# ltronchin/LatentAugment

Measured on NVIDIA B200. Metric: augmented images/sec, higher is better.
Workload: dtype bf16 operands, f32 accumulate

## Files before the change

latentaugment_b200/csrc/kernels.cu:

```cuda
#include "kernels.cuh"

#include <cuda_bf16.h>

#include "act.cuh"
#include "sm100.cuh"

namespace la {

namespace {

__device__ __forceinline__ float warp_sum(float v) {
#pragma unroll
    for (int o = 16; o >= 1; o >>= 1) v += __shfl_xor_sync(0xffffffffu, v, o);
    return v;
}
__device__ __forceinline__ double warp_sum_d(double v) {
#pragma unroll
    for (int o = 16; o >= 1; o >>= 1) v += __shfl_xor_sync(0xffffffffu, v, o);
    return v;
}
__device__ __forceinline__ void split_store(__nv_bfloat16* hi, __nv_bfloat16* lo, long long i, float v) {
    const __nv_bfloat16 h = __float2bfloat16_rn(v);
    hi[i] = h;
    if (lo) lo[i] = __float2bfloat16_rn(v - __bfloat162float(h));
// ... 185 lines not shown
__global__ void const_modulate_kernel(const float* __restrict__ c_f32, const float* __restrict__ s0, int batch, int hw, int C,
                                      __nv_bfloat16* hi, __nv_bfloat16* lo) {
    const long long idx = blockIdx.x * static_cast<long long>(blockDim.x) + threadIdx.x;
    if (idx >= static_cast<long long>(batch) * hw * C) return;
    const int c = static_cast<int>(idx % C);
    const int p = static_cast<int>((idx / C) % hw);
    const int n = static_cast<int>(idx / (static_cast<long long>(C) * hw));
    split_store(hi, lo, idx, c_f32[p * C + c] * s0[static_cast<long long>(n) * C + c]);
}

__device__ __forceinline__ unsigned pack2(float a, float b) {
    __nv_bfloat162 v = __floats2bfloat162_rn(a, b);
    return *reinterpret_cast<unsigned*>(&v);
}
__device__ __forceinline__ void st_bf16x2(unsigned* hi, unsigned* lo, long long i, float a, float b) {
    hi[i] = pack2(a, b);
    if (lo) lo[i] = pack2(a - __bfloat162float(__float2bfloat16_rn(a)), b - __bfloat162float(__float2bfloat16_rn(b)));
}

constexpr int kFirSeg = 32;
template <bool FWD, bool SPLIT, bool SEP>
__global__ void __launch_bounds__(256, SEP ? 3 : 2) upfir_slide_kernel(const __grid_constant__ UpFirParams P, int cpb, int chan_blocks) {
    const int hc = P.C >> 1;
    const int rows_per_block = 256 / cpb;
    const int cb = blockIdx.z % chan_blocks, n = blockIdx.z / chan_blocks;
    const int cp = cb * cpb + threadIdx.x % cpb;
    const int r = blockIdx.y * rows_per_block + threadIdx.x / cpb;
    const int x0 = blockIdx.x * kFirSeg;
    const int TW = P.OW + 1;
    const int out_h = FWD ? P.OH : P.TH, out_w = FWD ? P.OW : TW, out_pitch = FWD ? P.OW : P.TWp;
    const int src_h = FWD ? P.TH : P.OH, src_w = FWD ? TW : P.OW, src_pitch = FWD ? P.TWp : P.OW;
    if (r >= out_h) return;
    const int org = FWD ? -1 : -2;
    const unsigned* sh = reinterpret_cast<const unsigned*>(FWD ? P.t_hi : P.gy_hi);
    const unsigned* sl = reinterpret_cast<const unsigned*>(FWD ? P.t_lo : P.gy_lo);
    float wk[16], wy[4], wx[4];
#pragma unroll
    for (int k = 0; k < 16; ++k) wk[k] = FWD ? P.fk[k] : P.fk[15 - k];
#pragma unroll
    for (int k = 0; k < 4; ++k) { wy[k] = FWD ? P.fy[k] : P.fy[3 - k]; wx[k] = FWD ? P.fx[k] : P.fx[3 - k]; }
    long long rowoff[4];
    float rowmask[4];
#pragma unroll
    for (int k = 0; k < 4; ++k) {
        const int sr = r + org + k;
        const bool ok = sr >= 0 && sr < src_h;
        rowoff[k] = ((static_cast<long long>(n) * src_h + (ok ? sr : 0)) * src_pitch) * hc + cp;
        rowmask[k] = ok ? 1.f : 0.f;
    }
    float2 win[SEP ? 1 : 4][7];
    auto load_col = [&](int slot, int sc) {
        const bool cok = sc >= 0 && sc < src_w;
        const long long coff = static_cast<long long>(cok ? sc : 0) * hc;
        unsigned u[4], l[4];
#pragma unroll
        for (int k = 0; k < 4; ++k) {
            u[k] = __ldg(sh + rowoff[k] + coff);
            if (SPLIT) l[k] = __ldg(sl + rowoff[k] + coff);
        }
        float2 colsum = make_float2(0.f, 0.f);
#pragma unroll
        for (int k = 0; k < 4; ++k) {
            float2 v = make_float2(__uint_as_float(u[k] << 16), __uint_as_float(u[k] & 0xffff0000u));
            if (SPLIT) { v.x += __uint_as_float(l[k] << 16); v.y += __uint_as_float(l[k] & 0xffff0000u); }
            if (SEP) {
                const float m = wy[k] * rowmask[k];
                colsum.x = fmaf(m, v.x, colsum.x);
                colsum.y = fmaf(m, v.y, colsum.y);
            } else {
                const float m = cok ? rowmask[k] : 0.f;
                win[k][slot] = make_float2(v.x * m, v.y * m);
            }
        }
        if (SEP) win[0][slot] = cok ? colsum : make_float2(0.f, 0.f);
    };
#pragma unroll
    for (int k = 0; k < 3; ++k) load_col(k, x0 + org + k);

    float2 dm = make_float2(0.f, 0.f), bs = dm, sn = dm;
    const float* nrow = nullptr;
    if (FWD && !P.act_saved) {
        const int c = 2 * cp;
        dm = __ldg(reinterpret_cast<const float2*>(P.demod + static_cast<long long>(n) * P.C + c));
        bs = __ldg(reinterpret_cast<const float2*>(P.bias + c));
        if (P.s_next) sn = __ldg(reinterpret_cast<const float2*>(P.s_next + static_cast<long long>(n) * P.C + c));
        if (P.noise) nrow = P.noise + n * P.noise_stride_n + static_cast<long long>(r) * P.OW;
    }
    unsigned* oh = reinterpret_cast<unsigned*>(FWD ? P.x_hi : P.gt_hi);
    unsigned* ol = SPLIT ? reinterpret_cast<unsigned*>(FWD ? P.x_lo : P.gt_lo) : nullptr;
    unsigned* xsh = reinterpret_cast<unsigned*>(P.xs_hi);
    unsigned* xsl = SPLIT ? reinterpret_cast<unsigned*>(P.xs_lo) : nullptr;
    const long long obase = ((static_cast<long long>(n) * out_h + r) * out_pitch) * hc + cp;

#pragma unroll 1
    for (int xb = 0; xb < kFirSeg; xb += 4) {
        if (x0 + xb >= out_w) break;
#pragma unroll
        for (int u = 0; u < 4; ++u) load_col(3 + u, x0 + xb + org + 3 + u);
        float nzv[4];
#pragma unroll
        for (int u = 0; u < 4; ++u) nzv[u] = (FWD && nrow && x0 + xb + u < out_w) ? __ldg(nrow + x0 + xb + u) * P.noise_scale : 0.f;
#pragma unroll
        for (int u = 0; u < 4; ++u) {
            const int x = x0 + xb + u;
            if (x >= out_w) continue;
            float a0 = 0.f, a1 = 0.f;
            if (SEP) {
#pragma unroll
                for (int kx = 0; kx < 4; ++kx) {
                    a0 = fmaf(wx[kx], win[0][u + kx].x, a0);
                    a1 = fmaf(wx[kx], win[0][u + kx].y, a1);
                }
            } else {
#pragma unroll
                for (int ky = 0; ky < 4; ++ky)
#pragma unroll
                    for (int kx = 0; kx < 4; ++kx) {
                        const float2 v = win[ky][u + kx];
                        a0 = fmaf(wk[ky * 4 + kx], v.x, a0);
                        a1 = fmaf(wk[ky * 4 + kx], v.y, a1);
                    }
            }
            const long long o = obase + static_cast<long long>(x) * hc;
            if (FWD && P.act_saved) {
                const unsigned sv = __ldg(reinterpret_cast<const unsigned*>(P.act_saved) + o);
                const unsigned svl = P.act_saved_lo ? __ldg(reinterpret_cast<const unsigned*>(P.act_saved_lo) + o) : 0u;
                const float s0 = __uint_as_float(sv << 16) + __uint_as_float(svl << 16);
                const float s1 = __uint_as_float(sv & 0xffff0000u) + __uint_as_float(svl & 0xffff0000u);
                const float thr = act_saved_clamp(P.act_clamp, P.act_saved_lo != nullptr);
                const float g0 = act_grad(a0 * P.act_gain, s0, P.act_slope, thr), g1 = act_grad(a1 * P.act_gain, s1, P.act_slope, thr);
                st_bf16x2(oh, ol, o, g0, g1);
            } else if (FWD) {
                float z0 = fmaf(a0, dm.x, nzv[u]) + bs.x, z1 = fmaf(a1, dm.y, nzv[u]) + bs.y;
                z0 = (z0 > 0.f ? z0 : z0 * P.act_slope) * P.act_gain;
                z1 = (z1 > 0.f ? z1 : z1 * P.act_slope) * P.act_gain;
                if (P.act_clamp >= 0.f) {
                    z0 = fminf(fmaxf(z0, -P.act_clamp), P.act_clamp);
                    z1 = fminf(fmaxf(z1, -P.act_clamp), P.act_clamp);
                }
                st_bf16x2(oh, ol, o, z0, z1);
                if (P.s_next) st_bf16x2(xsh, xsl, o, z0 * sn.x, z1 * sn.y);
            } else {
                st_bf16x2(oh, ol, o, a0, a1);
            }
        }
#pragma unroll
        for (int ky = 0; ky < (SEP ? 1 : 4); ++ky)
#pragma unroll
            for (int k = 0; k < 3; ++k) win[ky][k] = win[ky][4 + k];
    }
}

constexpr int kFirRing = 8, kFirStrip = 32, kFirSlotBytes = 4608, kFirInPx = 35;
template <bool FWD>
__global__ void __launch_bounds__(160) upfir_tma_kernel(const __grid_constant__ UpFirParams P, int rows_per_cta, int nslabs) {
    extern __shared__ __align__(128) uint8_t fsm[];
    uint8_t* ring = fsm;
    uint8_t* stage = fsm + kFirRing * kFirSlotBytes;
    uint64_t* full = reinterpret_cast<uint64_t*>(stage + 4 * 2 * 2 * 1024);
    uint64_t* empty = full + kFirRing;
    const int warp = threadIdx.x >> 5, lane = threadIdx.x & 31;
    const int slab = blockIdx.y % nslabs, rblk = blockIdx.y / nslabs;
    const int n = blockIdx.z;
    const int x0 = blockIdx.x * kFirStrip;
    const int out_h = FWD ? P.OH : P.TH;
    const int r0 = rblk * rows_per_cta, r1 = min(r0 + rows_per_cta, out_h);
    const int org = FWD ? -1 : -2;
    const int c0 = slab * 64;
    const CUtensorMap* in_map = FWD ? &P.fwd_in : &P.bwd_in;
    if (threadIdx.x == 0) {
        for (int s = 0; s < kFirRing; ++s) { mbar_init(&full[s], 1); mbar_init(&empty[s], 4); }
        fence_barrier_init();
        prefetch_tmap(in_map);
    }
    __syncthreads();
    const int nrows_in = (r1 - r0) + 3;
    if (warp == 4) {
        if (lane == 0) {
            for (int j = 0; j < nrows_in; ++j) {
                const int s = j % kFirRing;
                mbar_wait(&empty[s], ((j / kFirRing) & 1) ^ 1, nullptr, 0);
                mbar_expect_tx(&full[s], kFirInPx * 128);
                tma_load_4d(ring + s * kFirSlotBytes, in_map, &full[s], c0, x0 + org, r0 + org + j, n);
            }
        }
        return;
    }
    float wy[4], wx[4];
#pragma unroll
    for (int k = 0; k < 4; ++k) { wy[k] = FWD ? P.fy[k] : P.fy[3 - k]; wx[k] = FWD ? P.fx[k] : P.fx[3 - k]; }
    float2 dm = make_float2(0.f, 0.f), bs = dm, sn = dm;
    const int c = c0 + 2 * lane;
    if (FWD && !P.act_saved) {
        dm = __ldg(reinterpret_cast<const float2*>(P.demod + static_cast<long long>(n) * P.C + c));
        bs = __ldg(reinterpret_cast<const float2*>(P.bias + c));
        if (P.s_next) sn = __ldg(reinterpret_cast<const float2*>(P.s_next + static_cast<long long>(n) * P.C + c));
    }
    const float clampv = P.act_clamp >= 0.f ? P.act_clamp : __int_as_float(0x7f800000);
    const float saved_thr = act_saved_clamp(P.act_clamp, false);
    const int px0 = warp * 8;
    uint8_t* my_stage = stage + warp * 4096;
    if constexpr (!FWD) {
        float2 ha[8], hb[8], hc[8], hd[8];
        auto hpass = [&](int j, float2 (&h)[8]) {
            mbar_wait(&full[j % kFirRing], (j / kFirRing) & 1, nullptr, 0);
            const unsigned* row = reinterpret_cast<const unsigned*>(ring + (j % kFirRing) * kFirSlotBytes) + px0 * 32 + lane;
            float2 in[11];
#pragma unroll
            for (int q = 0; q < 11; ++q) {
                const unsigned u = row[q * 32];
                in[q] = make_float2(__uint_as_float(u << 16), __uint_as_float(u & 0xffff0000u));
            }
            __syncwarp();
            if (lane == 0) mbar_arrive(&empty[j % kFirRing]);
#pragma unroll
            for (int i = 0; i < 8; ++i) {
                float a0 = wx[0] * in[i].x, a1 = wx[0] * in[i].y;
#pragma unroll
                for (int k = 1; k < 4; ++k) { a0 = fmaf(wx[k], in[i + k].x, a0); a1 = fmaf(wx[k], in[i + k].y, a1); }
                h[i] = make_float2(a0, a1);
            }
        };
        auto out_row = [&](int r, const float2 (&h0)[8], const float2 (&h1)[8], const float2 (&h2)[8], float2 (&h3)[8]) {
            const int j0 = r - r0;
            hpass(j0 + 3, h3);
            float nzv[8];
            unsigned svv[8];
            if (FWD && P.act_saved) {
                const unsigned* sp = reinterpret_cast<const unsigned*>(P.act_saved) +
                                     ((static_cast<long long>(n) * P.OH + r) * P.OW) * (P.C >> 1) + (c0 >> 1) + lane;
#pragma unroll
                for (int i = 0; i < 8; ++i) {
                    const int x = x0 + px0 + i;
                    svv[i] = x < P.OW ? __ldg(sp + static_cast<long long>(x) * (P.C >> 1)) : 0u;
                }
            }
            if (FWD && P.noise && !P.act_saved) {
                const float4* np = reinterpret_cast<const float4*>(P.noise + n * P.noise_stride_n + static_cast<long long>(r) * P.OW + x0 + px0);
                const bool in = x0 + px0 + 8 <= P.OW;
                const float4 a = in ? __ldg(np) : make_float4(0.f, 0.f, 0.f, 0.f), b = in ? __ldg(np + 1) : a;
                nzv[0] = a.x; nzv[1] = a.y; nzv[2] = a.z; nzv[3] = a.w; nzv[4] = b.x; nzv[5] = b.y; nzv[6] = b.z; nzv[7] = b.w;
#pragma unroll
                for (int i = 0; i < 8; ++i) nzv[i] *= P.noise_scale;
            } else {
#pragma unroll
                for (int i = 0; i < 8; ++i) nzv[i] = 0.f;
            }
            uint8_t* sx = my_stage + (j0 & 1) * 2048;
            if (lane == 0) bulk_wait_read<1>();
            __syncwarp();
#pragma unroll
            for (int i = 0; i < 8; ++i) {
                const float a0 = fmaf(wy[3], h3[i].x, fmaf(wy[2], h2[i].x, fmaf(wy[1], h1[i].x, wy[0] * h0[i].x)));
                const float a1 = fmaf(wy[3], h3[i].y, fmaf(wy[2], h2[i].y, fmaf(wy[1], h1[i].y, wy[0] * h0[i].y)));
                if (FWD && P.act_saved) {
                    const float s0 = __uint_as_float(svv[i] << 16), s1 = __uint_as_float(svv[i] & 0xffff0000u);
                    const float g0 = act_grad(a0 * P.act_gain, s0, P.act_slope, saved_thr);
                    const float g1 = act_grad(a1 * P.act_gain, s1, P.act_slope, saved_thr);
                    reinterpret_cast<unsigned*>(sx)[i * 32 + lane] = pack2(g0, g1);
                } else if (FWD) {
                    float z0 = fmaf(a0, dm.x, nzv[i]) + bs.x, z1 = fmaf(a1, dm.y, nzv[i]) + bs.y;
                    z0 = (z0 > 0.f ? z0 : z0 * P.act_slope) * P.act_gain;
                    z1 = (z1 > 0.f ? z1 : z1 * P.act_slope) * P.act_gain;
                    z0 = fminf(fmaxf(z0, -clampv), clampv);
                    z1 = fminf(fmaxf(z1, -clampv), clampv);
                    reinterpret_cast<unsigned*>(sx)[i * 32 + lane] = pack2(z0, z1);
                    reinterpret_cast<unsigned*>(sx + 1024)[i * 32 + lane] = pack2(z0 * sn.x, z1 * sn.y);
                } else {
                    reinterpret_cast<unsigned*>(sx)[i * 32 + lane] = pack2(a0, a1);
                }
            }
            fence_proxy_async();
            __syncwarp();
            if (lane == 0) {
                if (FWD) {
                    tma_store_4d(&P.fwd_out_x, sx, c0, x0 + px0, r, n);
                    if (P.s_next && !P.act_saved) tma_store_4d(&P.fwd_out_xs, sx + 1024, c0, x0 + px0, r, n);
                } else {
                    tma_store_4d(&P.bwd_out, sx, c0, x0 + px0, r, n);
                }
                bulk_commit();
            }
        };
        if (r0 < r1) { hpass(0, ha); hpass(1, hb); hpass(2, hc); }
        for (int r = r0; r < r1; r += 4) {
            out_row(r, ha, hb, hc, hd);
            if (r + 1 < r1) out_row(r + 1, hb, hc, hd, ha);
            if (r + 2 < r1) out_row(r + 2, hc, hd, ha, hb);
            if (r + 3 < r1) out_row(r + 3, hd, ha, hb, hc);
        }
    } else {
        for (int j = 0; j < 3; ++j) mbar_wait(&full[j % kFirRing], (j / kFirRing) & 1, nullptr, 0);
        for (int r = r0; r < r1; ++r) {
            const int j0 = r - r0;
            mbar_wait(&full[(j0 + 3) % kFirRing], ((j0 + 3) / kFirRing) & 1, nullptr, 0);
            float2 cs[11];
#pragma unroll
            for (int q = 0; q < 11; ++q) cs[q] = make_float2(0.f, 0.f);
#pragma unroll
            for (int k = 0; k < 4; ++k) {
                const unsigned* row = reinterpret_cast<const unsigned*>(ring + ((j0 + k) % kFirRing) * kFirSlotBytes) + px0 * 32 + lane;
#pragma unroll
                for (int q = 0; q < 11; ++q) {
                    const unsigned u = row[q * 32];
                    cs[q].x = fmaf(wy[k], __uint_as_float(u << 16), cs[q].x);
                    cs[q].y = fmaf(wy[k], __uint_as_float(u & 0xffff0000u), cs[q].y);
                }
            }
            __syncwarp();
            if (lane == 0) mbar_arrive(&empty[j0 % kFirRing]);
            float nzv[8];
            unsigned svv[8];
            if (FWD && P.act_saved) {
                const unsigned* sp = reinterpret_cast<const unsigned*>(P.act_saved) +
                                     ((static_cast<long long>(n) * P.OH + r) * P.OW) * (P.C >> 1) + (c0 >> 1) + lane;
#pragma unroll
                for (int i = 0; i < 8; ++i) {
                    const int x = x0 + px0 + i;
                    svv[i] = x < P.OW ? __ldg(sp + static_cast<long long>(x) * (P.C >> 1)) : 0u;
                }
            }
            if (FWD && P.noise && !P.act_saved) {
                const float4* np = reinterpret_cast<const float4*>(P.noise + n * P.noise_stride_n + static_cast<long long>(r) * P.OW + x0 + px0);
                const bool in = x0 + px0 + 8 <= P.OW;
                const float4 a = in ? __ldg(np) : make_float4(0.f, 0.f, 0.f, 0.f), b = in ? __ldg(np + 1) : a;
                nzv[0] = a.x; nzv[1] = a.y; nzv[2] = a.z; nzv[3] = a.w; nzv[4] = b.x; nzv[5] = b.y; nzv[6] = b.z; nzv[7] = b.w;
#pragma unroll
                for (int i = 0; i < 8; ++i) nzv[i] *= P.noise_scale;
            } else {
#pragma unroll
                for (int i = 0; i < 8; ++i) nzv[i] = 0.f;
            }
            uint8_t* sx = my_stage + (j0 & 1) * 2048;
            if (lane == 0) bulk_wait_read<1>();
            __syncwarp();
#pragma unroll
            for (int i = 0; i < 8; ++i) {
                float a0 = 0.f, a1 = 0.f;
#pragma unroll
                for (int k = 0; k < 4; ++k) { a0 = fmaf(wx[k], cs[i + k].x, a0); a1 = fmaf(wx[k], cs[i + k].y, a1); }
                if (FWD && P.act_saved) {
                    const float s0 = __uint_as_float(svv[i] << 16), s1 = __uint_as_float(svv[i] & 0xffff0000u);
                    const float g0 = act_grad(a0 * P.act_gain, s0, P.act_slope, saved_thr);
                    const float g1 = act_grad(a1 * P.act_gain, s1, P.act_slope, saved_thr);
                    reinterpret_cast<unsigned*>(sx)[i * 32 + lane] = pack2(g0, g1);
                } else if (FWD) {
                    float z0 = fmaf(a0, dm.x, nzv[i]) + bs.x, z1 = fmaf(a1, dm.y, nzv[i]) + bs.y;
                    z0 = (z0 > 0.f ? z0 : z0 * P.act_slope) * P.act_gain;
                    z1 = (z1 > 0.f ? z1 : z1 * P.act_slope) * P.act_gain;
                    z0 = fminf(fmaxf(z0, -clampv), clampv);
                    z1 = fminf(fmaxf(z1, -clampv), clampv);
                    reinterpret_cast<unsigned*>(sx)[i * 32 + lane] = pack2(z0, z1);
                    reinterpret_cast<unsigned*>(sx + 1024)[i * 32 + lane] = pack2(z0 * sn.x, z1 * sn.y);
                } else {
                    reinterpret_cast<unsigned*>(sx)[i * 32 + lane] = pack2(a0, a1);
                }
            }
            fence_proxy_async();
            __syncwarp();
            if (lane == 0) {
                if (FWD) {
                    tma_store_4d(&P.fwd_out_x, sx, c0, x0 + px0, r, n);
                    if (P.s_next && !P.act_saved) tma_store_4d(&P.fwd_out_xs, sx + 1024, c0, x0 + px0, r, n);
                } else {
                    tma_store_4d(&P.bwd_out, sx, c0, x0 + px0, r, n);
                }
                bulk_commit();
            }
        }
    }
    if (lane == 0) bulk_wait_read<0>();
}

__device__ __forceinline__ void up_taps(int v, int lowres, int& i0, int& i1, float& c0, float& c1) {
    const int m = v >> 1;
    if (v & 1) { i0 = m; i1 = m + 1; c0 = 0.75f; c1 = 0.25f; }
    else { i0 = m - 1; i1 = m; c0 = 0.25f; c1 = 0.75f; }
    if (i0 < 0) { c0 = 0.f; i0 = 0; }
    if (i1 >= lowres) { c1 = 0.f; i1 = lowres - 1; }
}

__device__ __forceinline__ float4 f4_fma(float c, float4 a, float4 acc) {
    return make_float4(fmaf(c, a.x, acc.x), fmaf(c, a.y, acc.y), fmaf(c, a.z, acc.z), fmaf(c, a.w, acc.w));
}

__device__ __forceinline__ float4 rgb_preclamp(const float4* __restrict__ parts, int nparts, long long stride, long long pix,
                                               const float* __restrict__ bias, int img_c) {
    float4 t = make_float4(0.f, 0.f, 0.f, 0.f);
    for (int b = 0; b < nparts; ++b) {
        const float4 p = parts[b * stride + pix];
        t.x += p.x; t.y += p.y; t.z += p.z;
    }
    t.x += bias[0];
    if (img_c > 1) t.y += bias[1];
    if (img_c > 2) t.z += bias[2];
    return t;
}

__global__ void rgb_combine_kernel(const float4* __restrict__ parts, int nparts, const float* __restrict__ bias, int img_c,
                                   float clamp, const float4* __restrict__ img_low, int batch, int res, float4* img,
                                   float* out_nchw) {
    const long long pix = blockIdx.x * static_cast<long long>(blockDim.x) + threadIdx.x;
    const long long total = static_cast<long long>(batch) * res * res;
    if (pix >= total) return;
    float4 t = rgb_preclamp(parts, nparts, total, pix, bias, img_c);
    if (clamp >= 0.f) {
        t.x = fminf(fmaxf(t.x, -clamp), clamp);
        t.y = fminf(fmaxf(t.y, -clamp), clamp);
        t.z = fminf(fmaxf(t.z, -clamp), clamp);
    }
    const int w = static_cast<int>(pix % res), h = static_cast<int>((pix / res) % res);
    const int n = static_cast<int>(pix / (static_cast<long long>(res) * res));
    if (img_low) {
        const int lr = res >> 1;
        int y0, y1, x0, x1;
        float cy0, cy1, cx0, cx1;
        up_taps(h, lr, y0, y1, cy0, cy1);
        up_taps(w, lr, x0, x1, cx0, cx1);
        const float4* base = img_low + static_cast<long long>(n) * lr * lr;
        float4 u = make_float4(0.f, 0.f, 0.f, 0.f);
        u = f4_fma(cy0 * cx0, base[y0 * lr + x0], u);
        u = f4_fma(cy0 * cx1, base[y0 * lr + x1], u);
        u = f4_fma(cy1 * cx0, base[y1 * lr + x0], u);
        u = f4_fma(cy1 * cx1, base[y1 * lr + x1], u);
        t.x += u.x; t.y += u.y; t.z += u.z;
    }
    img[pix] = t;
    if (out_nchw) {
        const long long plane = static_cast<long long>(res) * res;
        float* o = out_nchw + static_cast<long long>(n) * img_c * plane + static_cast<long long>(h) * res + w;
        o[0] = t.x;
        if (img_c > 1) o[plane] = t.y;
        if (img_c > 2) o[2 * plane] = t.z;
    }
}

__global__ void rgb_backward_kernel(const float4* __restrict__ g_img, const float4* __restrict__ parts, int nparts,
                                    const float* __restrict__ bias, int img_c, float clamp, int batch, int res, float4* g_rgb,
                                    float4* g_img_low) {
    const long long pix = blockIdx.x * static_cast<long long>(blockDim.x) + threadIdx.x;
    const long long total = static_cast<long long>(batch) * res * res;
    if (pix >= total) return;
    const float4 g = g_img[pix];
    const float4 t = rgb_preclamp(parts, nparts, total, pix, bias, img_c);
    float4 r = g;
    if (clamp >= 0.f) {
        if (!(fabsf(t.x) <= clamp)) r.x = 0.f;
        if (!(fabsf(t.y) <= clamp)) r.y = 0.f;
        if (!(fabsf(t.z) <= clamp)) r.z = 0.f;
    }
    r.w = 0.f;
    g_rgb[pix] = r;
    if (g_img_low) {
        const int w = static_cast<int>(pix % res), h = static_cast<int>((pix / res) % res);
        if ((w | h) & 1) return;
        const int n = static_cast<int>(pix / (static_cast<long long>(res) * res));
        const int my = h >> 1, mx = w >> 1, lr = res >> 1;
        const float cf[4] = {0.25f, 0.75f, 0.75f, 0.25f};
        float4 acc = make_float4(0.f, 0.f, 0.f, 0.f);
        const float4* base = g_img + static_cast<long long>(n) * res * res;
        for (int a = 0; a < 4; ++a) {
            const int yy = 2 * my - 1 + a;
            if (yy < 0 || yy >= res) continue;
            for (int b = 0; b < 4; ++b) {
                const int xx = 2 * mx - 1 + b;
                if (xx < 0 || xx >= res) continue;
                acc = f4_fma(cf[a] * cf[b], base[static_cast<long long>(yy) * res + xx], acc);
            }
        }
        g_img_low[(static_cast<long long>(n) * lr + my) * lr + mx] = acc;
    }
}

__global__ void pix_loss_kernel(const float4* __restrict__ img, const float4* __restrict__ bank_mean, int batch, int res,
                                int img_c, int crop_off, int crop_size, float w_pix, float4* g_img, float* loss_parts) {
    const long long total = static_cast<long long>(batch) * res * res;
    const float gs = -(w_pix / img_c) * 2.f / (static_cast<float>(batch) * crop_size * crop_size);
    float acc = 0.f;
    for (long long pix = blockIdx.x * static_cast<long long>(blockDim.x) + threadIdx.x; pix < total;
         pix += static_cast<long long>(gridDim.x) * blockDim.x) {
        const int w = static_cast<int>(pix % res), h = static_cast<int>((pix / res) % res);
        float4 g = make_float4(0.f, 0.f, 0.f, 0.f);
        if (h >= crop_off && h < crop_off + crop_size && w >= crop_off && w < crop_off + crop_size) {
            const float4 x = img[pix];
            const float4 y = bank_mean[h * res + w];
            g.x = gs * (x.x - y.x);
            acc += x.x * x.x - 2.f * x.x * y.x;
            if (img_c > 1) { g.y = gs * (x.y - y.y); acc += x.y * x.y - 2.f * x.y * y.y; }
            if (img_c > 2) { g.z = gs * (x.z - y.z); acc += x.z * x.z - 2.f * x.z * y.z; }
        }
        g_img[pix] = g;
    }
    __shared__ float sm[32];
    acc = warp_sum(acc);
    if ((threadIdx.x & 31) == 0) sm[threadIdx.x >> 5] = acc;
    __syncthreads();
    if (threadIdx.x < 32) {
        float v = threadIdx.x < (blockDim.x >> 5) ? sm[threadIdx.x] : 0.f;
        v = warp_sum(v);
        if (threadIdx.x == 0) loss_parts[blockIdx.x] = v;
    }
}

__global__ void style_grad_rgb_kernel(LayerTable T, int batch, const float* __restrict__ red_rgb, float* g_s) {
    const RgbDesc D = T.rgb[blockIdx.y];
    const int i = blockIdx.x * blockDim.x + threadIdx.x;
    const int n = blockIdx.z;
    if (i >= D.cin) return;
    const float* rr = red_rgb + 3LL * batch * D.roff;
    const long long e = static_cast<long long>(n) * D.cin + i;
    const long long plane = static_cast<long long>(batch) * D.cin;
    float g = D.wt[i] * rr[e];
    if (D.img_c > 1) g += D.wt[D.cin + i] * rr[plane + e];
    if (D.img_c > 2) g += D.wt[2 * D.cin + i] * rr[2 * plane + e];
    g_s[static_cast<long long>(batch) * D.soff + e] = g;
}

constexpr int kGwRows = 64, kGwSamples = 4;
__global__ void gw_partial_kernel(const float* __restrict__ g_s, const float* __restrict__ a_cat, const int* __restrict__ chunk_soff,
                                  const int* __restrict__ chunk_cin, int batch, int w_dim, float* partial) {
// ... 99 lines not shown
    for (int k = threadIdx.x; k < w_dim; k += blockDim.x) {
        double acc = 0.0;
        for (int m = m0; m < m1; ++m)
            for (int j = 0; j < num_ws; ++j) {
                const double v = W[(static_cast<long long>(m) * num_ws + j) * w_dim + k];
                acc += v;
                sq += v * v;
            }
        psum[static_cast<long long>(blockIdx.x) * w_dim + k] = acc;
    }
    __shared__ double sm[32];
    sq = warp_sum_d(sq);
    if ((threadIdx.x & 31) == 0) sm[threadIdx.x >> 5] = sq;
    __syncthreads();
    if (threadIdx.x == 0) {
        double t = 0.0;
        for (int i = 0; i < (blockDim.x >> 5); ++i) t += sm[i];
        pm2[blockIdx.x] = t;
    }
}
__global__ void latent_bank_final_kernel(const double* __restrict__ psum, const double* __restrict__ pm2, int nblocks, int M,
                                         int w_dim, float* w_sum, float* m2) {
    for (int k = threadIdx.x; k < w_dim; k += blockDim.x) {
        double acc = 0.0;
        for (int b = 0; b < nblocks; ++b) acc += psum[static_cast<long long>(b) * w_dim + k];
        w_sum[k] = static_cast<float>(acc / M);
    }
    if (threadIdx.x == 0) {
        double t = 0.0;
        for (int b = 0; b < nblocks; ++b) t += pm2[b];
        m2[0] = static_cast<float>(t / M);
    }
}

__global__ void image_bank_mean_kernel(const float* __restrict__ X, int M, int C, int res, float4* mean) {
    const int p = blockIdx.x * blockDim.x + threadIdx.x;
    if (p >= res * res) return;
    float acc[3] = {0.f, 0.f, 0.f};
    const long long plane = static_cast<long long>(res) * res;
    for (int m = 0; m < M; ++m)
        for (int c = 0; c < C && c < 3; ++c) acc[c] += X[(static_cast<long long>(m) * C + c) * plane + p];
    mean[p] = make_float4(acc[0] / M, acc[1] / M, acc[2] / M, 0.f);
}
__global__ void image_bank_m2_kernel(const float* __restrict__ X, int M, int C, int res, int crop_off, int crop_size, float* m2) {
    const int c = blockIdx.x;
    const long long plane = static_cast<long long>(res) * res;
    const long long per = static_cast<long long>(crop_size) * crop_size;
    double acc = 0.0;
    for (long long e = threadIdx.x; e < per * M; e += blockDim.x) {
        const int m = static_cast<int>(e / per);
        const int q = static_cast<int>(e % per);
        const int h = crop_off + q / crop_size, w = crop_off + q % crop_size;
        const double v = X[(static_cast<long long>(m) * C + c) * plane + static_cast<long long>(h) * res + w];
        acc += v * v;
    }
    __shared__ double sm[32];
    acc = warp_sum_d(acc);
    if ((threadIdx.x & 31) == 0) sm[threadIdx.x >> 5] = acc;
    __syncthreads();
    if (threadIdx.x == 0) {
        double t = 0.0;
        for (int i = 0; i < (blockDim.x >> 5); ++i) t += sm[i];
        m2[c] = static_cast<float>(t / M);
    }
}

__global__ void mapping_normalize_kernel(const float* __restrict__ z, int z_dim, float* out) {
    const int n = blockIdx.x;
    float acc = 0.f;
    for (int k = threadIdx.x; k < z_dim; k += blockDim.x) { const float v = z[static_cast<long long>(n) * z_dim + k]; acc += v * v; }
    __shared__ float sm[32];
    acc = warp_sum(acc);
    if ((threadIdx.x & 31) == 0) sm[threadIdx.x >> 5] = acc;
    __syncthreads();
    float t = 0.f;
    for (int i = 0; i < (blockDim.x >> 5); ++i) t += sm[i];
    const float r = rsqrtf(t / z_dim + 1e-8f);
    for (int k = threadIdx.x; k < z_dim; k += blockDim.x) out[static_cast<long long>(n) * z_dim + k] = z[static_cast<long long>(n) * z_dim + k] * r;
}

__global__ void mapping_fc_kernel(const float* __restrict__ x, const float* __restrict__ w, const float* __restrict__ b, int batch,
                                  int n_in, int n_out, float w_gain, float b_gain, int lrelu, float* y) {
    const int j = blockIdx.x * (blockDim.x >> 5) + (threadIdx.x >> 5);
    const int lane = threadIdx.x & 31;
    if (j >= n_out) return;
    float a[kMaxRowRegs];
#pragma unroll
    for (int r = 0; r < kMaxRowRegs; ++r) a[r] = (lane + 32 * r < n_in) ? w[static_cast<long long>(j) * n_in + lane + 32 * r] * w_gain : 0.f;
    const float bj = b[j] * b_gain;
    for (int n = 0; n < batch; ++n) {
        float acc = 0.f;
#pragma unroll
        for (int r = 0; r < kMaxRowRegs; ++r)
            if (lane + 32 * r < n_in) acc = fmaf(a[r], x[static_cast<long long>(n) * n_in + lane + 32 * r], acc);
        acc = warp_sum(acc);
        if (lane == 0) {
            float v = acc + bj;
            if (lrelu) v = (v > 0.f ? v : 0.2f * v) * 1.41421356237309515f;
            y[static_cast<long long>(n) * n_out + j] = v;
        }
    }
}

__global__ void mapping_truncate_kernel(const float* __restrict__ w, const float* __restrict__ w_avg, float psi, int n, int w_dim,
                                        float* out) {
    const int e = blockIdx.x * blockDim.x + threadIdx.x;
    if (e >= n) return;
    const float a = w_avg[e % w_dim];
    out[e] = a + psi * (w[e] - a);
}

}

int prep_conv_weights(const float* w, int cout, int cin, int up, const float* fir4x4, int split, void* wf, void* wb, float* w2,
                      float* w2t, cudaStream_t s) {
    const long long n = static_cast<long long>(cout) * cin;
    prep_conv_weights_kernel<<<cdiv(n, 128), 128, 0, s>>>(w, cout, cin, up, fir4x4, split, static_cast<__nv_bfloat16*>(wf),
                                                          static_cast<__nv_bfloat16*>(wb), w2, w2t);
    return last_err();
}
int prep_affine(const float* aw, const float* ab, int cin, int w_dim, float wscale, float bscale, float* a_rows, float* b_rows,
                cudaStream_t s) {
    prep_affine_kernel<<<cdiv(static_cast<long long>(cin) * w_dim, 256), 256, 0, s>>>(aw, ab, cin, w_dim, wscale, bscale, a_rows, b_rows);
    return last_err();
}
__global__ void prep_axpy_kernel(const float* __restrict__ x, float a, float* y, long long n) {
    const long long i = blockIdx.x * static_cast<long long>(blockDim.x) + threadIdx.x;
    if (i < n) y[i] = fmaf(a, x[i], y[i]);
}
int prep_axpy(const float* x, float a, float* y, long long n, cudaStream_t s) {
    prep_axpy_kernel<<<cdiv(n, 256), 256, 0, s>>>(x, a, y, n);
    return last_err();
}
int prep_scale(const float* src, float scale, float* dst, long long n, cudaStream_t s) {
    prep_scale_kernel<<<cdiv(n, 256), 256, 0, s>>>(src, scale, dst, n);
    return last_err();
}
int prep_const(const float* cst, int C, int hw, float* c_f32, void* hi, void* lo, cudaStream_t s) {
    prep_const_kernel<<<cdiv(C * hw, 256), 256, 0, s>>>(cst, C, hw, c_f32, static_cast<__nv_bfloat16*>(hi), static_cast<__nv_bfloat16*>(lo));
    return last_err();
}

static int max_cin(const LayerTable& T, bool conv, bool rgb) {
    int m = 0;
    if (conv) for (int i = 0; i < T.nconv; ++i) m = T.conv[i].cin > m ? T.conv[i].cin : m;
    if (rgb) for (int i = 0; i < T.nrgb; ++i) m = T.rgb[i].cin > m ? T.rgb[i].cin : m;
    return m;
}

static int upfir_launch(const UpFirParams& p, bool fwd, cudaStream_t s) {
    if (p.use_tma) {
        const int smem = kFirRing * kFirSlotBytes + 4 * 2 * 2 * 1024 + 2 * kFirRing * 8;
        const int out_h = fwd ? p.OH : p.TH, out_w = fwd ? p.OW : p.OW + 1;
        const int nslabs = p.C / 64;
        const int strips = cdiv(out_w, kFirStrip);
        int rblocks = 1;
        while (static_cast<long long>(strips) * nslabs * p.B * rblocks < 148 * 6 && out_h / (rblocks * 2) >= 32) rblocks *= 2;
        const int rows_per_cta = cdiv(out_h, rblocks);
        dim3 grid(strips, nslabs * cdiv(out_h, rows_per_cta), p.B);
        if (fwd) {
            static bool a[kMaxDevices] = {};
            const int dev = current_device_slot();
            if (!a[dev]) { cudaFuncSetAttribute(upfir_tma_kernel<true>, cudaFuncAttributeMaxDynamicSharedMemorySize, smem); a[dev] = true; }
            upfir_tma_kernel<true><<<grid, 160, smem, s>>>(p, rows_per_cta, nslabs);
        } else {
            static bool a[kMaxDevices] = {};
            const int dev = current_device_slot();
            if (!a[dev]) { cudaFuncSetAttribute(upfir_tma_kernel<false>, cudaFuncAttributeMaxDynamicSharedMemorySize, smem); a[dev] = true; }
            upfir_tma_kernel<false><<<grid, 160, smem, s>>>(p, rows_per_cta, nslabs);
        }
        return last_err();
    }
    const int hc = p.C / 2;
    int cpb = hc < 256 ? hc : 256;
    if (256 % cpb || hc % cpb) return static_cast<int>(cudaErrorInvalidValue);
    const int chan_blocks = hc / cpb, rows_per_block = 256 / cpb;
    const int out_h = fwd ? p.OH : p.TH, out_w = fwd ? p.OW : p.OW + 1;
    dim3 grid(cdiv(out_w, kFirSeg), cdiv(out_h, rows_per_block), p.B * chan_blocks);
#define LA_FIR(F, S, Q) upfir_slide_kernel<F, S, Q><<<grid, 256, 0, s>>>(p, cpb, chan_blocks)
    const int sel = (fwd ? 4 : 0) | (p.split ? 2 : 0) | (p.separable ? 1 : 0);
    switch (sel) {
        case 0: LA_FIR(false, false, false); break;
        case 1: LA_FIR(false, false, true); break;
        case 2: LA_FIR(false, true, false); break;
        case 3: LA_FIR(false, true, true); break;
        case 4: LA_FIR(true, false, false); break;
        case 5: LA_FIR(true, false, true); break;
        case 6: LA_FIR(true, true, false); break;
        default: LA_FIR(true, true, true); break;
    }
#undef LA_FIR
    return last_err();
}
int upfir_forward(const UpFirParams& p, cudaStream_t s) { return upfir_launch(p, true, s); }
int upfir_backward(const UpFirParams& p, cudaStream_t s) { return upfir_launch(p, false, s); }

int styles_forward(const LayerTable& T, const float* ws, long long sn, long long sidx, const float* a_cat, const float* b_cat,
                   int w_dim, int batch, float* s_cat, cudaStream_t s) {
    StyleGemmArgs A{};
    A.ws = ws; A.sn = sn; A.sidx = sidx; A.a_cat = a_cat; A.b_cat = b_cat; A.w_dim = w_dim; A.out = s_cat;
    dim3 grid(cdiv(max_cin(T, true, true), kSgRows), T.nconv + T.nrgb, cdiv(batch, kSgSamples));
    style_gemm_kernel<kSgStyles><<<grid, 128, 0, s>>>(T, batch, A);
    return last_err();
}
int demod_rgbw_forward(const LayerTable& T, int batch, const float* s_cat, float* d_cat, float4* rgbw, cudaStream_t s) {
    int mco = 0;
    for (int i = 0; i < T.nconv; ++i) mco = T.conv[i].cout > mco ? T.conv[i].cout : mco;
    StyleGemmArgs A{};
    A.s_cat = s_cat; A.out = d_cat;
    style_gemm_kernel<kSgDemod><<<dim3(cdiv(mco, kSgRows), T.nconv, cdiv(batch, kSgSamples)), 128, 0, s>>>(T, batch, A);
    int e = last_err();
    if (e) return e;
    rgbw_kernel<<<dim3(cdiv(max_cin(T, false, true), 128), T.nrgb, batch), 128, 0, s>>>(T, batch, s_cat, rgbw);
    return last_err();
}
int const_modulate(const float* c_f32, const float* s0, int batch, int hw, int C, int split, void* xs_hi, void* xs_lo, cudaStream_t s) {
    const long long n = static_cast<long long>(batch) * hw * C;
    const_modulate_kernel<<<cdiv(n, 256), 256, 0, s>>>(c_f32, s0, batch, hw, C, static_cast<__nv_bfloat16*>(xs_hi),
                                                        split ? static_cast<__nv_bfloat16*>(xs_lo) : nullptr);
    return last_err();
}
int rgb_combine(const float4* parts, int nparts, const float* bias, int img_c, float clamp, const float4* img_low, int batch, int res,
                float4* img, float* out_nchw, cudaStream_t s) {
    const long long n = static_cast<long long>(batch) * res * res;
    rgb_combine_kernel<<<cdiv(n, 256), 256, 0, s>>>(parts, nparts, bias, img_c, clamp, img_low, batch, res, img, out_nchw);
    return last_err();
}
int rgb_backward(const float4* g_img, const float4* parts, int nparts, const float* bias, int img_c, float clamp, int batch, int res,
                 float4* g_rgb, float4* g_img_low, cudaStream_t s) {
    const long long n = static_cast<long long>(batch) * res * res;
    rgb_backward_kernel<<<cdiv(n, 256), 256, 0, s>>>(g_img, parts, nparts, bias, img_c, clamp, batch, res, g_rgb, g_img_low);
    return last_err();
}
int pix_loss(const float4* img, const float4* bank_mean, const float* , int batch, int res, int img_c, int crop_off,
             int crop_size, float w_pix, float4* g_img, float* loss_parts, int* nparts_out, cudaStream_t s) {
    const long long n = static_cast<long long>(batch) * res * res;
    int grid = cdiv(n, 256);
    if (grid > 1024) grid = 1024;
    pix_loss_kernel<<<grid, 256, 0, s>>>(img, bank_mean, batch, res, img_c, crop_off, crop_size, w_pix, g_img, loss_parts);
    *nparts_out = grid;
    return last_err();
}
int style_grad(const LayerTable& T, int batch, const float* s_cat, const float* d_cat, const float* red_s, const float* red_d,
               const float* red_rgb, float* g_s, cudaStream_t s) {
    int mco = 0;
    for (int i = 0; i < T.nconv; ++i) mco = T.conv[i].cout > mco ? T.conv[i].cout : mco;
    (void)mco;
    StyleGemmArgs A{};
    A.s_cat = s_cat; A.d_cat = d_cat; A.red_s = red_s; A.red_d = red_d; A.out = g_s;
    style_gemm_kernel<kSgGrad><<<dim3(cdiv(max_cin(T, true, false), kSgRows), T.nconv, cdiv(batch, kSgSamples)), 128, 0, s>>>(T, batch, A);
    int e = last_err();
    if (e) return e;
    style_grad_rgb_kernel<<<dim3(cdiv(max_cin(T, false, true), 128), T.nrgb, batch), 128, 0, s>>>(T, batch, red_rgb, g_s);
    return last_err();
}
int gw_partial(const float* g_s, const float* a_cat, const int* chunk_soff, const int* chunk_cin, int nchunks, int batch, int w_dim,
               float* partial, cudaStream_t s) {
    gw_partial_kernel<<<dim3(nchunks, cdiv(batch, kGwSamples)), 256, 0, s>>>(g_s, a_cat, chunk_soff, chunk_cin, batch, w_dim, partial);
    return last_err();
}
int adam_step(const float* partial, int nchunks, int use_partial, const float* w_sum_bank, const float* lat_m2, const AdamConsts* consts, int* step_counter,
              float* w, float* m, float* v, int batch, int w_dim, const float* pix_parts, int n_pix_parts, const float* bank_m2,
              int img_c, int crop_size, float* loss_log, int max_steps, const float* disc_loss, const float* lpips_loss, cudaStream_t s) {
    loss_value_kernel<<<1, 512, 0, s>>>(w, w_sum_bank, lat_m2, consts, step_counter, batch, w_dim, pix_parts, n_pix_parts, bank_m2, img_c,
                                        crop_size, loss_log, max_steps, disc_loss, lpips_loss);
    adam_kernel<<<cdiv(batch * w_dim, 256), 256, 0, s>>>(partial, nchunks, use_partial, w_sum_bank, consts, step_counter, w, m, v, batch, w_dim);
    step_inc_kernel<<<1, 1, 0, s>>>(step_counter);
    return last_err();
}
int finalize_w(const float* w_opt, const float* w0, float alpha, int soft, int batch, int w_dim, float* w_aug, cudaStream_t s) {
    finalize_w_kernel<<<cdiv(batch * w_dim, 256), 256, 0, s>>>(w_opt, w0, alpha, soft, batch * w_dim, w_aug);
    return last_err();
}

int latent_bank_stats(const float* W, int M, int num_ws, int w_dim, float* w_sum, float* m2, cudaStream_t s) {
    double* scratch = nullptr;
    const int nb = M < kBankBlocks ? M : kBankBlocks;
    cudaError_t e = cudaMallocAsync(&scratch, sizeof(double) * (static_cast<size_t>(nb) * w_dim + nb), s);
    if (e != cudaSuccess) return static_cast<int>(e);
    latent_bank_partial_kernel<<<nb, 256, 0, s>>>(W, M, num_ws, w_dim, scratch, scratch + static_cast<size_t>(nb) * w_dim);
    latent_bank_final_kernel<<<1, 256, 0, s>>>(scratch, scratch + static_cast<size_t>(nb) * w_dim, nb, M, w_dim, w_sum, m2);
    int r = last_err();
    cudaFreeAsync(scratch, s);
    return r;
}
int image_bank_stats(const float* X, int M, int C, int res, int crop_off, int crop_size, float4* mean, float* m2, cudaStream_t s) {
    image_bank_mean_kernel<<<cdiv(res * res, 256), 256, 0, s>>>(X, M, C, res, mean);
    image_bank_m2_kernel<<<C < 3 ? C : 3, 1024, 0, s>>>(X, M, C, res, crop_off, crop_size, m2);
    return last_err();
}

int mapping_normalize(const float* z, int batch, int z_dim, float* out, cudaStream_t s) {
    mapping_normalize_kernel<<<batch, 256, 0, s>>>(z, z_dim, out);
    return last_err();
}
int mapping_fc(const float* x, const float* w, const float* b, int batch, int n_in, int n_out, float w_gain, float b_gain, int lrelu,
               float* y, cudaStream_t s) {
    if (n_in > 32 * kMaxRowRegs) return static_cast<int>(cudaErrorInvalidValue);
    mapping_fc_kernel<<<cdiv(n_out, 4), 128, 0, s>>>(x, w, b, batch, n_in, n_out, w_gain, b_gain, lrelu, y);
    return last_err();
}
int mapping_truncate(const float* w, const float* w_avg, float psi, int batch, int w_dim, float* out, cudaStream_t s) {
    mapping_truncate_kernel<<<cdiv(batch * w_dim, 256), 256, 0, s>>>(w, w_avg, psi, batch * w_dim, w_dim, out);
    return last_err();
}

}
```

Baseline: 378.9.

## Make TMA upfir kernel persistent with work-item walk and register-ring vertical FIR

Converts the TMA-fed upsample FIR kernel into a persistent kernel. A grid sized to resident CTAs strides over (row-run, strip, slab, batch) items, and the producer's mbarrier ring runs continuously across items. The forward path now keeps rolling vertical partial sums in registers, so each input row is read from shared memory once instead of four times. The act_saved case becomes a template parameter, and row-run length adapts to occupancy. Each item re-primes 3 halo rows, and register pressure rises under the 3-blocks launch bound.

```diff
diff --git a/latentaugment_b200/csrc/kernels.cu b/latentaugment_b200/csrc/kernels.cu
--- a/latentaugment_b200/csrc/kernels.cu
+++ b/latentaugment_b200/csrc/kernels.cu
@@ -361,21 +361,17 @@
 }
 
 constexpr int kFirRing = 8, kFirStrip = 32, kFirSlotBytes = 4608, kFirInPx = 35;
-template <bool FWD>
-__global__ void __launch_bounds__(160) upfir_tma_kernel(const __grid_constant__ UpFirParams P, int rows_per_cta, int nslabs) {
+struct FirWalk { int rows, runs, strips, nslabs, items; };
+template <bool FWD, bool ACT>
+__global__ void __launch_bounds__(160, 3) upfir_tma_kernel(const __grid_constant__ UpFirParams P, const FirWalk W) {
     extern __shared__ __align__(128) uint8_t fsm[];
     uint8_t* ring = fsm;
     uint8_t* stage = fsm + kFirRing * kFirSlotBytes;
     uint64_t* full = reinterpret_cast<uint64_t*>(stage + 4 * 2 * 2 * 1024);
     uint64_t* empty = full + kFirRing;
     const int warp = threadIdx.x >> 5, lane = threadIdx.x & 31;
-    const int slab = blockIdx.y % nslabs, rblk = blockIdx.y / nslabs;
-    const int n = blockIdx.z;
-    const int x0 = blockIdx.x * kFirStrip;
     const int out_h = FWD ? P.OH : P.TH;
-    const int r0 = rblk * rows_per_cta, r1 = min(r0 + rows_per_cta, out_h);
     const int org = FWD ? -1 : -2;
-    const int c0 = slab * 64;
     const CUtensorMap* in_map = FWD ? &P.fwd_in : &P.bwd_in;
     if (threadIdx.x == 0) {
         for (int s = 0; s < kFirRing; ++s) { mbar_init(&full[s], 1); mbar_init(&empty[s], 4); }
@@ -383,14 +379,30 @@
         prefetch_tmap(in_map);
     }
     __syncthreads();
-    const int nrows_in = (r1 - r0) + 3;
+    struct Item { int r0, r1, x0, c0, n; };
+    auto item_at = [&](int it) {
+        Item I;
+        const int run = it % W.runs;
+        it /= W.runs;
+        I.x0 = (it % W.strips) * kFirStrip;
+        it /= W.strips;
+        I.c0 = (it % W.nslabs) * 64;
+        I.n = it / W.nslabs;
+        I.r0 = run * W.rows;
+        I.r1 = min(I.r0 + W.rows, out_h);
+        return I;
+    };
+    uint32_t g = 0;
     if (warp == 4) {
         if (lane == 0) {
-            for (int j = 0; j < nrows_in; ++j) {
-                const int s = j % kFirRing;
-                mbar_wait(&empty[s], ((j / kFirRing) & 1) ^ 1, nullptr, 0);
-                mbar_expect_tx(&full[s], kFirInPx * 128);
-                tma_load_4d(ring + s * kFirSlotBytes, in_map, &full[s], c0, x0 + org, r0 + org + j, n);
+            for (int it = blockIdx.x; it < W.items; it += gridDim.x) {
+                const Item I = item_at(it);
+                for (int j = 0; j < I.r1 - I.r0 + 3; ++j, ++g) {
+                    const int s = g % kFirRing;
+                    mbar_wait(&empty[s], ((g / kFirRing) & 1) ^ 1, nullptr, 0);
+                    mbar_expect_tx(&full[s], kFirInPx * 128);
+                    tma_load_4d(ring + s * kFirSlotBytes, in_map, &full[s], I.c0, I.x0 + org, I.r0 + org + j, I.n);
+                }
             }
         }
         return;
@@ -398,44 +410,34 @@
     float wy[4], wx[4];
 #pragma unroll
     for (int k = 0; k < 4; ++k) { wy[k] = FWD ? P.fy[k] : P.fy[3 - k]; wx[k] = FWD ? P.fx[k] : P.fx[3 - k]; }
-    float2 dm = make_float2(0.f, 0.f), bs = dm, sn = dm;
-    const int c = c0 + 2 * lane;
-    if (FWD && !P.act_saved) {
-        dm = __ldg(reinterpret_cast<const float2*>(P.demod + static_cast<long long>(n) * P.C + c));
-        bs = __ldg(reinterpret_cast<const float2*>(P.bias + c));
-        if (P.s_next) sn = __ldg(reinterpret_cast<const float2*>(P.s_next + static_cast<long long>(n) * P.C + c));
-    }
     const float clampv = P.act_clamp >= 0.f ? P.act_clamp : __int_as_float(0x7f800000);
     const float saved_thr = act_saved_clamp(P.act_clamp, false);
     const int px0 = warp * 8;
     uint8_t* my_stage = stage + warp * 4096;
-    if constexpr (!FWD) {
-        float2 ha[8], hb[8], hc[8], hd[8];
-        auto hpass = [&](int j, float2 (&h)[8]) {
-            mbar_wait(&full[j % kFirRing], (j / kFirRing) & 1, nullptr, 0);
-            const unsigned* row = reinterpret_cast<const unsigned*>(ring + (j % kFirRing) * kFirSlotBytes) + px0 * 32 + lane;
-            float2 in[11];
-#pragma unroll
-            for (int q = 0; q < 11; ++q) {
-                const unsigned u = row[q * 32];
-                in[q] = make_float2(__uint_as_float(u << 16), __uint_as_float(u & 0xffff0000u));
-            }
-            __syncwarp();
-            if (lane == 0) mbar_arrive(&empty[j % kFirRing]);
-#pragma unroll
-            for (int i = 0; i < 8; ++i) {
-                float a0 = wx[0] * in[i].x, a1 = wx[0] * in[i].y;
-#pragma unroll
-                for (int k = 1; k < 4; ++k) { a0 = fmaf(wx[k], in[i + k].x, a0); a1 = fmaf(wx[k], in[i + k].y, a1); }
-                h[i] = make_float2(a0, a1);
-            }
-        };
-        auto out_row = [&](int r, const float2 (&h0)[8], const float2 (&h1)[8], const float2 (&h2)[8], float2 (&h3)[8]) {
-            const int j0 = r - r0;
-            hpass(j0 + 3, h3);
+    uint32_t st = 0;
+    auto take_row = [&](unsigned (&u)[11]) {
+        mbar_wait(&full[g % kFirRing], (g / kFirRing) & 1, nullptr, 0);
+        const unsigned* row = reinterpret_cast<const unsigned*>(ring + (g % kFirRing) * kFirSlotBytes) + px0 * 32 + lane;
+#pragma unroll
+        for (int q = 0; q < 11; ++q) u[q] = row[q * 32];
+        __syncwarp();
+        if (lane == 0) mbar_arrive(&empty[g % kFirRing]);
+        ++g;
+    };
+    for (int it = blockIdx.x; it < W.items; it += gridDim.x) {
+        const Item I = item_at(it);
+        const int r0 = I.r0, r1 = I.r1, x0 = I.x0, c0 = I.c0, n = I.n;
+        auto store_row = [&](int r, const float2 (&a)[8]) {
+            float2 dm = make_float2(0.f, 0.f), bs = dm, sn = dm;
+            if (FWD && !ACT) {
+                const int c = c0 + 2 * lane;
+                dm = __ldg(reinterpret_cast<const float2*>(P.demod + static_cast<long long>(n) * P.C + c));
+                bs = __ldg(reinterpret_cast<const float2*>(P.bias + c));
+                if (P.s_next) sn = __ldg(reinterpret_cast<const float2*>(P.s_next + static_cast<long long>(n) * P.C + c));
+            }
             float nzv[8];
             unsigned svv[8];
-            if (FWD && P.act_saved) {
+            if (ACT) {
                 const unsigned* sp = reinterpret_cast<const unsigned*>(P.act_saved) +
                                      ((static_cast<long long>(n) * P.OH + r) * P.OW) * (P.C >> 1) + (c0 >> 1) + lane;
 #pragma unroll
@@ -444,25 +446,25 @@
                     svv[i] = x < P.OW ? __ldg(sp + static_cast<long long>(x) * (P.C >> 1)) : 0u;
                 }
             }
-            if (FWD && P.noise && !P.act_saved) {
+            if (FWD && !ACT && P.noise) {
                 const float4* np = reinterpret_cast<const float4*>(P.noise + n * P.noise_stride_n + static_cast<long long>(r) * P.OW + x0 + px0);
                 const bool in = x0 + px0 + 8 <= P.OW;
-                const float4 a = in ? __ldg(np) : make_float4(0.f, 0.f, 0.f, 0.f), b = in ? __ldg(np + 1) : a;
-                nzv[0] = a.x; nzv[1] = a.y; nzv[2] = a.z; nzv[3] = a.w; nzv[4] = b.x; nzv[5] = b.y; nzv[6] = b.z; nzv[7] = b.w;
+                const float4 a4 = in ? __ldg(np) : make_float4(0.f, 0.f, 0.f, 0.f), b4 = in ? __ldg(np + 1) : a4;
+                nzv[0] = a4.x; nzv[1] = a4.y; nzv[2] = a4.z; nzv[3] = a4.w; nzv[4] = b4.x; nzv[5] = b4.y; nzv[6] = b4.z; nzv[7] = b4.w;
 #pragma unroll
                 for (int i = 0; i < 8; ++i) nzv[i] *= P.noise_scale;
             } else {
 #pragma unroll
                 for (int i = 0; i < 8; ++i) nzv[i] = 0.f;
             }
-            uint8_t* sx = my_stage + (j0 & 1) * 2048;
+            uint8_t* sx = my_stage + (st & 1) * 2048;
+            ++st;
             if (lane == 0) bulk_wait_read<1>();
             __syncwarp();
 #pragma unroll
             for (int i = 0; i < 8; ++i) {
-                const float a0 = fmaf(wy[3], h3[i].x, fmaf(wy[2], h2[i].x, fmaf(wy[1], h1[i].x, wy[0] * h0[i].x)));
-                const float a1 = fmaf(wy[3], h3[i].y, fmaf(wy[2], h2[i].y, fmaf(wy[1], h1[i].y, wy[0] * h0[i].y)));
-                if (FWD && P.act_saved) {
+                const float a0 = a[i].x, a1 = a[i].y;
+                if (ACT) {
                     const float s0 = __uint_as_float(svv[i] << 16), s1 = __uint_as_float(svv[i] & 0xffff0000u);
                     const float g0 = act_grad(a0 * P.act_gain, s0, P.act_slope, saved_thr);
                     const float g1 = act_grad(a1 * P.act_gain, s1, P.act_slope, saved_thr);
@@ -484,97 +486,93 @@
             if (lane == 0) {
                 if (FWD) {
                     tma_store_4d(&P.fwd_out_x, sx, c0, x0 + px0, r, n);
-                    if (P.s_next && !P.act_saved) tma_store_4d(&P.fwd_out_xs, sx + 1024, c0, x0 + px0, r, n);
+                    if (!ACT && P.s_next) tma_store_4d(&P.fwd_out_xs, sx + 1024, c0, x0 + px0, r, n);
                 } else {
                     tma_store_4d(&P.bwd_out, sx, c0, x0 + px0, r, n);
                 }
                 bulk_commit();
             }
         };
-        if (r0 < r1) { hpass(0, ha); hpass(1, hb); hpass(2, hc); }
-        for (int r = r0; r < r1; r += 4) {
-            out_row(r, ha, hb, hc, hd);
-            if (r + 1 < r1) out_row(r + 1, hb, hc, hd, ha);
-            if (r + 2 < r1) out_row(r + 2, hc, hd, ha, hb);
-            if (r + 3 < r1) out_row(r + 3, hd, ha, hb, hc);
-        }
-    } else {
-        for (int j = 0; j < 3; ++j) mbar_wait(&full[j % kFirRing], (j / kFirRing) & 1, nullptr, 0);
-        for (int r = r0; r < r1; ++r) {
-            const int j0 = r - r0;
-            mbar_wait(&full[(j0 + 3) % kFirRing], ((j0 + 3) / kFirRing) & 1, nullptr, 0);
-            float2 cs[11];
-#pragma unroll
-            for (int q = 0; q < 11; ++q) cs[q] = make_float2(0.f, 0.f);
-#pragma unroll
-            for (int k = 0; k < 4; ++k) {
-                const unsigned* row = reinterpret_cast<const unsigned*>(ring + ((j0 + k) % kFirRing) * kFirSlotBytes) + px0 * 32 + lane;
+        if constexpr (!FWD) {
+            float2 ha[8], hb[8], hc[8], hd[8];
+            auto hpass = [&](float2 (&h)[8]) {
+                unsigned u[11];
+                take_row(u);
+#pragma unroll
+                for (int i = 0; i < 8; ++i) {
+                    float a0 = wx[0] * __uint_as_float(u[i] << 16), a1 = wx[0] * __uint_as_float(u[i] & 0xffff0000u);
+#pragma unroll
+                    for (int k = 1; k < 4; ++k) {
+                        a0 = fmaf(wx[k], __uint_as_float(u[i + k] << 16), a0);
+                        a1 = fmaf(wx[k], __uint_as_float(u[i + k] & 0xffff0000u), a1);
+                    }
+                    h[i] = make_float2(a0, a1);
+                }
+            };
+            auto out_row = [&](int r, const float2 (&h0)[8], const float2 (&h1)[8], const float2 (&h2)[8], float2 (&h3)[8]) {
+                hpass(h3);
+                float2 a[8];
+#pragma unroll
+                for (int i = 0; i < 8; ++i) {
+                    a[i].x = fmaf(wy[3], h3[i].x, fmaf(wy[2], h2[i].x, fmaf(wy[1], h1[i].x, wy[0] * h0[i].x)));
+                    a[i].y = fmaf(wy[3], h3[i].y, fmaf(wy[2], h2[i].y, fmaf(wy[1], h1[i].y, wy[0] * h0[i].y)));
+                }
+                store_row(r, a);
+            };
+            hpass(ha); hpass(hb); hpass(hc);
+            for (int r = r0; r < r1; r += 4) {
+                out_row(r, ha, hb, hc, hd);
+                if (r + 1 < r1) out_row(r + 1, hb, hc, hd, ha);
+                if (r + 2 < r1) out_row(r + 2, hc, hd, ha, hb);
+                if (r + 3 < r1) out_row(r + 3, hd, ha, hb, hc);
+            }
+        } else {
+            float2 pa[11], pb[11], pc[11];
+            auto tap = [&](float2 (&p)[11], const unsigned (&u)[11], float w) {
 #pragma unroll
                 for (int q = 0; q < 11; ++q) {
-                    const unsigned u = row[q * 32];
-                    cs[q].x = fmaf(wy[k], __uint_as_float(u << 16), cs[q].x);
-                    cs[q].y = fmaf(wy[k], __uint_as_float(u & 0xffff0000u), cs[q].y);
+                    p[q].x = fmaf(w, __uint_as_float(u[q] << 16), p[q].x);
+                    p[q].y = fmaf(w, __uint_as_float(u[q] & 0xffff0000u), p[q].y);
                 }
-            }
-            __syncwarp();
-            if (lane == 0) mbar_arrive(&empty[j0 % kFirRing]);
-            float nzv[8];
-            unsigned svv[8];
-            if (FWD && P.act_saved) {
-                const unsigned* sp = reinterpret_cast<const unsigned*>(P.act_saved) +
-                                     ((static_cast<long long>(n) * P.OH + r) * P.OW) * (P.C >> 1) + (c0 >> 1) + lane;
+            };
+            auto open = [&](float2 (&p)[11], const unsigned (&u)[11]) {
+#pragma unroll
+                for (int q = 0; q < 11; ++q)
+                    p[q] = make_float2(fmaf(wy[0], __uint_as_float(u[q] << 16), 0.f), fmaf(wy[0], __uint_as_float(u[q] & 0xffff0000u), 0.f));
+            };
+            auto out_row = [&](int r, float2 (&p3)[11], float2 (&p2)[11], float2 (&p1)[11]) {
+                unsigned u[11];
+                take_row(u);
+                tap(p3, u, wy[3]);
+                tap(p2, u, wy[2]);
+                tap(p1, u, wy[1]);
+                float2 a[8];
 #pragma unroll
                 for (int i = 0; i < 8; ++i) {
-                    const int x = x0 + px0 + i;
-                    svv[i] = x < P.OW ? __ldg(sp + static_cast<long long>(x) * (P.C >> 1)) : 0u;
+                    float a0 = 0.f, a1 = 0.f;
+#pragma unroll
+                    for (int k = 0; k < 4; ++k) { a0 = fmaf(wx[k], p3[i + k].x, a0); a1 = fmaf(wx[k], p3[i + k].y, a1); }
+                    a[i] = make_float2(a0, a1);
                 }
-            }
-            if (FWD && P.noise && !P.act_saved) {
-                const float4* np = reinterpret_cast<const float4*>(P.noise + n * P.noise_stride_n + static_cast<long long>(r) * P.OW + x0 + px0);
-                const bool in = x0 + px0 + 8 <= P.OW;
-                const float4 a = in ? __ldg(np) : make_float4(0.f, 0.f, 0.f, 0.f), b = in ? __ldg(np + 1) : a;
-                nzv[0] = a.x; nzv[1] = a.y; nzv[2] = a.z; nzv[3] = a.w; nzv[4] = b.x; nzv[5] = b.y; nzv[6] = b.z; nzv[7] = b.w;
-#pragma unroll
-                for (int i = 0; i < 8; ++i) nzv[i] *= P.noise_scale;
-            } else {
-#pragma unroll
-                for (int i = 0; i < 8; ++i) nzv[i] = 0.f;
-            }
-            uint8_t* sx = my_stage + (j0 & 1) * 2048;
-            if (lane == 0) bulk_wait_read<1>();
-            __syncwarp();
-#pragma unroll
-            for (int i = 0; i < 8; ++i) {
-                float a0 = 0.f, a1 = 0.f;
-#pragma unroll
-                for (int k = 0; k < 4; ++k) { a0 = fmaf(wx[k], cs[i + k].x, a0); a1 = fmaf(wx[k], cs[i + k].y, a1); }
-                if (FWD && P.act_saved) {
-                    const float s0 = __uint_as_float(svv[i] << 16), s1 = __uint_as_float(svv[i] & 0xffff0000u);
-                    const float g0 = act_grad(a0 * P.act_gain, s0, P.act_slope, saved_thr);
-                    const float g1 = act_grad(a1 * P.act_gain, s1, P.act_slope, saved_thr);
-                    reinterpret_cast<unsigned*>(sx)[i * 32 + lane] = pack2(g0, g1);
-                } else if (FWD) {
-                    float z0 = fmaf(a0, dm.x, nzv[i]) + bs.x, z1 = fmaf(a1, dm.y, nzv[i]) + bs.y;
-                    z0 = (z0 > 0.f ? z0 : z0 * P.act_slope) * P.act_gain;
-                    z1 = (z1 > 0.f ? z1 : z1 * P.act_slope) * P.act_gain;
-                    z0 = fminf(fmaxf(z0, -clampv), clampv);
-                    z1 = fminf(fmaxf(z1, -clampv), clampv);
-                    reinterpret_cast<unsigned*>(sx)[i * 32 + lane] = pack2(z0, z1);
-                    reinterpret_cast<unsigned*>(sx + 1024)[i * 32 + lane] = pack2(z0 * sn.x, z1 * sn.y);
-                } else {
-                    reinterpret_cast<unsigned*>(sx)[i * 32 + lane] = pack2(a0, a1);
-                }
-            }
-            fence_proxy_async();
-            __syncwarp();
-            if (lane == 0) {
-                if (FWD) {
-                    tma_store_4d(&P.fwd_out_x, sx, c0, x0 + px0, r, n);
-                    if (P.s_next && !P.act_saved) tma_store_4d(&P.fwd_out_xs, sx + 1024, c0, x0 + px0, r, n);
-                } else {
-                    tma_store_4d(&P.bwd_out, sx, c0, x0 + px0, r, n);
-                }
-                bulk_commit();
+                store_row(r, a);
+                open(p3, u);
+            };
+            {
+                unsigned u[11];
+                take_row(u);
+                open(pa, u);
+                take_row(u);
+                tap(pa, u, wy[1]);
+                open(pb, u);
+                take_row(u);
+                tap(pa, u, wy[2]);
+                tap(pb, u, wy[1]);
+                open(pc, u);
+            }
+            for (int r = r0; r < r1; r += 3) {
+                out_row(r, pa, pb, pc);
+                if (r + 1 < r1) out_row(r + 1, pb, pc, pa);
+                if (r + 2 < r1) out_row(r + 2, pc, pa, pb);
             }
         }
     }
@@ -980,23 +978,29 @@
     if (p.use_tma) {
         const int smem = kFirRing * kFirSlotBytes + 4 * 2 * 2 * 1024 + 2 * kFirRing * 8;
         const int out_h = fwd ? p.OH : p.TH, out_w = fwd ? p.OW : p.OW + 1;
-        const int nslabs = p.C / 64;
-        const int strips = cdiv(out_w, kFirStrip);
-        int rblocks = 1;
-        while (static_cast<long long>(strips) * nslabs * p.B * rblocks < 148 * 6 && out_h / (rblocks * 2) >= 32) rblocks *= 2;
-        const int rows_per_cta = cdiv(out_h, rblocks);
-        dim3 grid(strips, nslabs * cdiv(out_h, rows_per_cta), p.B);
-        if (fwd) {
-            static bool a[kMaxDevices] = {};
-            const int dev = current_device_slot();
-            if (!a[dev]) { cudaFuncSetAttribute(upfir_tma_kernel<true>, cudaFuncAttributeMaxDynamicSharedMemorySize, smem); a[dev] = true; }
-            upfir_tma_kernel<true><<<grid, 160, smem, s>>>(p, rows_per_cta, nslabs);
-        } else {
-            static bool a[kMaxDevices] = {};
-            const int dev = current_device_slot();
-            if (!a[dev]) { cudaFuncSetAttribute(upfir_tma_kernel<false>, cudaFuncAttributeMaxDynamicSharedMemorySize, smem); a[dev] = true; }
-            upfir_tma_kernel<false><<<grid, 160, smem, s>>>(p, rows_per_cta, nslabs);
-        }
+        const int mode = fwd ? (p.act_saved ? 2 : 1) : 0;
+        void (*kern)(UpFirParams, FirWalk) = mode == 2 ? upfir_tma_kernel<true, true>
+                                             : (mode == 1 ? upfir_tma_kernel<true, false> : upfir_tma_kernel<false, false>);
+        static int slots[3][kMaxDevices] = {};
+        int& resident = slots[mode][current_device_slot()];
+        if (!resident) {
+            int dev = 0, sms = 0, per_sm = 0;
+            cudaGetDevice(&dev);
+            cudaDeviceGetAttribute(&sms, cudaDevAttrMultiProcessorCount, dev);
+            cudaFuncSetAttribute(kern, cudaFuncAttributeMaxDynamicSharedMemorySize, smem);
+            cudaOccupancyMaxActiveBlocksPerMultiprocessor(&per_sm, kern, 160, smem);
+            if (sms * per_sm <= 0) { const int e = last_err(); return e ? e : static_cast<int>(cudaErrorLaunchOutOfResources); }
+            resident = sms * per_sm;
+        }
+        FirWalk W;
+        W.strips = cdiv(out_w, kFirStrip);
+        W.nslabs = p.C / 64;
+        W.rows = 64;
+        const long long tiles = static_cast<long long>(W.strips) * W.nslabs * p.B;
+        while (W.rows > 8 && tiles * cdiv(out_h, W.rows) < 8LL * resident) W.rows /= 2;
+        W.runs = cdiv(out_h, W.rows);
+        W.items = static_cast<int>(tiles * W.runs);
+        kern<<<W.items < resident ? W.items : resident, 160, smem, s>>>(p, W);
         return last_err();
     }
     const int hc = p.C / 2;
```

New measurement: 381.6, median of 6. No clear change (+0.7%).
